# shuoli0708/LRS-PnP-DIP

Measured on AMD Instinct MI355X. Metric: PnP-ISTA+DIP iters/sec on 200×200×198 HSI cube; MPSNR vs reference, higher is better.
Workload: dtype f32 (MFMA products fp32-accurate) + f64 (NLM prox, BN/sigma statistics)

## Files before the change

### include/lrspnp.h

```cpp
#ifndef LRSPNP_H
#define LRSPNP_H

#include <stddef.h>
#include <stdint.h>

#ifdef __cplusplus
extern "C" {
#endif

#define LRS_OK 0
#define LRS_E_INVALID (-1)
#define LRS_E_UNSUPPORTED (-2)
#define LRS_E_WORKSPACE (-3)
#define LRS_E_NODEVICE (-4)

#define LRS_ALPHA_SPEC2 0
#define LRS_ALPHA_FRO4 1
#define LRS_ALPHA_SOFT 2
#define LRS_PROX_NLM 0
#define LRS_PROX_SOFT 1
#define LRS_PROX_NLM_MATLAB 2

const char *lrs_version(void);
int lrs_check_device(void);

int lrs_nlm_col_f32(const float *g, int64_t ldg, float *out, int64_t ldo, int64_t K, int64_t nvec,
                    double h, const double *h_per_vec, int patch_size, int patch_distance,
                    void *stream);

int64_t lrs_block_count(int64_t P, int64_t B, int64_t bb, int64_t sliding);
int lrs_block_grid(int64_t P, int64_t B, int64_t bb, int64_t sliding, int32_t *rows, int32_t *cols,
                   int64_t nb);
int lrs_cover_ranges(int64_t extent, int64_t bb, const int32_t *starts, int64_t nstarts,
                     int32_t *lo, int32_t *hi);

int lrs_im2col_f32(const float *X, const float *L, float mu, int64_t P, int64_t B, int64_t bb,
                   const int32_t *rows, const int32_t *cols, int64_t nb, int64_t n_pad, float *Yb,
                   uint8_t *obs, void *stream);

size_t lrs_ista_alpha_workspace(int64_t n, int64_t K, int64_t npat);
int lrs_ista_alpha_f32(const float *D, int64_t n, int64_t K, const uint8_t *obs_pat, int64_t npat,
                       int64_t n_pad, int alpha_mode, float lambda_ista, float *alpha_pat,
                       double *thr_pat, void *ws, size_t ws_bytes, void *stream);

#define LRS_ISTA_F32 0
#define LRS_ISTA_SPLIT_BF16 1
#define LRS_ISTA_ALGO_AUTO 0
#define LRS_ISTA_ALGO_GENERIC 1
typedef struct {
    int32_t precision;
    int32_t max_workgroups;
    int32_t algorithm;
    int32_t warm_start;
    int32_t reserved[4];
} lrs_ista_opts;
size_t lrs_ista_workspace(int64_t n, int64_t K, int prox, const lrs_ista_opts *opts);
int lrs_ista_f32(const float *Yb, const uint8_t *obs, const float *D, int64_t n, int64_t n_pad,
                 int64_t K, int64_t nb, const float *alpha, const double *thr, int Nit, int prox,
                 float *coefs, float *phi, const lrs_ista_opts *opts, void *ws, size_t ws_bytes,
                 void *stream);
int64_t lrs_ista_pat_plan_len(int64_t nb, int64_t npat);
int64_t lrs_ista_pat_plan(const int32_t *pat, int64_t nb, int64_t npat, int32_t *plan, int64_t cap);
int lrs_ista_pat_preferred(int64_t n, int64_t K, int64_t nb, int64_t npat, int Nit);
size_t lrs_ista_pat_workspace(int64_t n, int64_t K, int64_t npat);
int lrs_ista_pat_prepare(const float *D, int64_t n, int64_t K, const uint8_t *obs_pat, int64_t npat,
                         int64_t n_pad, void *ws, size_t ws_bytes, void *stream);
int lrs_ista_pat_f32(const float *Yb, const uint8_t *obs_pat, int64_t npat, const int32_t *plan,
                     int64_t ntiles, int64_t n, int64_t n_pad, int64_t K, int64_t nb,
                     const float *alpha, const double *thr, int Nit, int prox, float *coefs, float *phi,
                     const lrs_ista_opts *opts, void *ws, size_t ws_bytes, void *stream);
size_t lrs_dict_workspace(int64_t n, int64_t n_pad, int64_t K, int64_t nb);
int lrs_dict_stats_f32(const float *coefs, int64_t nb, int64_t K, float *H, double *c, void *ws,
                       size_t ws_bytes, void *stream);
int lrs_dict_update_f32(const float *Yb, const uint8_t *obs, const float *coefs, float *D, int64_t n,
                        int64_t n_pad, int64_t K, int64_t nb, const double *c, int n_inner, double *obj,
                        void *ws, size_t ws_bytes, void *stream);
int lrs_dict_normalise_f32(float *D, int64_t n, int64_t K, void *stream);
int lrs_nlm_matlab_col_f32(const float *g, int64_t ldg, float *out, int64_t ldo, int64_t K,
                           int64_t nvec, double h, const double *h_per_vec, void *stream);
#define LRS_DIP_F32 0
#define LRS_DIP_SPLIT_BF16 1
typedef struct {
    int32_t precision;
    int32_t upsample_dgrad;
    int32_t reserved[6];
} lrs_dip_opts;

#define LRS_SVT_WARM 1
#define LRS_SVT_JACOBI 2
#define LRS_SVT_MULTI_WG 4
#define LRS_SVT_WIDE_TRI 8
#define LRS_SVT_WIDE_MW 16
int64_t lrs_svt_max_bands(void);
size_t lrs_svt_workspace(int64_t P, int64_t B);
int lrs_svt_f32(const float *X, const float *L2, float c2, int64_t P, int64_t B, double tau,
                float *U, double *s_out, int warm, void *ws, size_t ws_bytes, void *stream);
int lrs_svt_gram_f32(const float *X, const float *L2, float c2, int64_t P, int64_t B, int warm,
                     void *ws, size_t ws_bytes, void *stream);
int lrs_svt_finish_f32(const float *X, const float *L2, float c2, int64_t P, int64_t B, double tau,
                       float *U, double *s_out, int warm, void *ws, size_t ws_bytes, void *stream);
int lrs_svt_gram_offset(int64_t P, int64_t B, int64_t *offset_bytes, int64_t *ld);

int lrs_admm_update_f32(float *X, float *L1, float *L2, const float *Y, const float *M,
                        const float *U, const float *phi, int64_t P, int64_t B, int64_t bb,
                        int64_t n_pad, const int32_t *row_starts, const int32_t *col_starts,
                        int64_t nbr, const int32_t *rlo, const int32_t *rhi, const int32_t *clo,
                        const int32_t *chi, float gamma, float mu1, float mu2, double *norms,
                        float *imout, void *stream);

#define LRS_PAD_ZERO 0
#define LRS_PAD_REFLECT 1
#define LRS_ACT_NONE 0
#define LRS_ACT_LRELU 1
#define LRS_ACT_SIGMOID 2

int lrs_conv2d_out_size(int H, int W, int k, int stride, int pad, int upsample, int *Ho, int *Wo);
int64_t lrs_conv2d_col_size(int Cin, int H, int W, int k, int stride, int pad, int upsample);
size_t lrs_conv2d_workspace(int Cin, int H, int W, int Cout, int k, int stride, int pad, int upsample,
                            const lrs_dip_opts *opts);
int lrs_conv2d_fwd_f32(const float *x, int Cin, int H, int W, const float *w, const float *bias,
                       int Cout, int k, int stride, int pad, int pad_mode, int upsample, float *col,
                       float *y, const lrs_dip_opts *opts, void *ws, size_t ws_bytes, void *stream);
int lrs_conv2d_bwd_f32(const float *gy, const float *col, const float *w, const float *w_div, int Cin,
                       int H, int W, int Cout, int k, int stride, int pad, int pad_mode, int upsample,
                       float *gx, float *gw, const lrs_dip_opts *opts, void *ws, size_t ws_bytes,
                       void *stream);
int lrs_conv2d_bwd_x_f32(const float *gy, const float *x, const float *w, const float *w_div, int Cin,
                         int H, int W, int Cout, int k, int stride, int pad, int pad_mode, int upsample,
                         float *gx, float *gw, const lrs_dip_opts *opts, void *ws, size_t ws_bytes,
                         void *stream);

size_t lrs_bn_act_workspace(int C, int64_t P);
int lrs_bn_act_fwd_f32(const float *z, float *y, const float *gamma, const float *beta, float *mean,
                       float *invstd, float *run_mean, float *run_var, int C, int64_t P, int act,
                       float eps, float momentum, void *ws, size_t ws_bytes, void *stream);
int lrs_bn_act_bwd_f32(const float *gy, const float *y, const float *z, const float *gamma,
                       const float *mean, const float *invstd, float *gz, float *ggamma,
                       float *gbeta, float *gbias, int C, int64_t P, int act, void *ws, size_t ws_bytes,
                       void *stream);
int lrs_conv_bn_small_f32(const float *x, int Cin, int H, int W, const float *w, const float *bias, int Cout,
                          int k, int stride, int pad, int pad_mode, int upsample, const float *gamma,
                          const float *beta, int lip, int act, float *z, float *y, float *mean, float *invstd,
                          float *run_mean, float *run_var, void *stream);

size_t lrs_sigma_max_workspace(int n);
int lrs_sigma_max_f32(const float *const *W, float *const *Wn, const int *rows, const int *cols, int n,
                      float ln_lambda, float *sigma, float *scale, void *ws, size_t ws_bytes,
                      void *stream);

int lrs_adam_f32(float *p, const float *g, float *m, float *v, int64_t n, const int *step, float lr,
                 float beta1, float beta2, float eps, void *stream);
int lrs_masked_mse_f32(const float *out, const float *target, const float *mask, int C, int64_t P,
                       float *gout, double *loss_acc, void *stream);
int lrs_masked_mse_cmask_f32(const float *out, const float *target, const float *mask, int mask_channels,
                             int C, int64_t P, float *gout, double *loss_acc, void *stream);
int lrs_masked_mse_framed_f32(const float *out, const float *target, const float *mask, int mask_channels,
                              int C, int64_t P, int64_t n_mean, float *gout, double *loss_acc, void *stream);

int lrs_unfolded_to_image_f32(const float *X, const float *L, float c, int64_t H, int64_t W, int64_t B,
                              float *img, void *stream);
int lrs_image_to_unfolded_f32(const float *img, int64_t H, int64_t W, int64_t B, float *X, void *stream);
int lrs_unfolded_to_frame_f32(const float *X, const float *L, float c, int64_t H, int64_t W, int64_t B,
                              int64_t top, int64_t left, int64_t Hf, int64_t Wf, float *img, void *stream);
int lrs_frame_to_unfolded_f32(const float *img, int64_t H, int64_t W, int64_t B, int64_t top, int64_t left,
                              int64_t Hf, int64_t Wf, float *X, void *stream);

typedef struct {
    int32_t count, size, patience, wait, stop, stop_epoch, best_epoch, reserved;
// ... 64 lines not shown
```

### lrs-pnp-dip_amd/csrc/dip_launch.h

```cpp
#pragma once
#include <math.h>
#include <string.h>

#include <algorithm>
#include <new>
#include <vector>

#include "dip_kernels.h"
#include "dip_bn.h"
#include "dip_sn.h"
#include "dip_train.h"
#include "dip_gemm.h"
#include "dip_pw.h"
#include "dip_wprep.h"
#include "dip_dgrad.h"
#include "dip_sm.h"
#include "dip_dir.h"
#include "dip_image.h"
#include "ista_paths.h"

using namespace lrs;

namespace {

constexpr int kEw = 256;
constexpr int64_t kForkBigP = 9604;

inline unsigned ew_blocks(int64_t n, int64_t cap = 4096) {
    int64_t b = (n + kEw - 1) / kEw;
    if (b < 1) b = 1;
    if (b > cap) b = cap;
    return (unsigned)b;
}

inline lrs_dip_opts dip_opts(const lrs_dip_opts *o) {
    lrs_dip_opts d{};
    d.precision = LRS_DIP_SPLIT_BF16;
    d.upsample_dgrad = 0;
    return o ? *o : d;
}
inline bool dip_opts_ok(const lrs_dip_opts &o) {
    return (o.precision == LRS_DIP_F32 || o.precision == LRS_DIP_SPLIT_BF16) && (o.upsample_dgrad == 0 || o.upsample_dgrad == 1);
}

int make_geom(int Cin, int H, int W, int k, int stride, int pad, int pad_mode, int up, ConvGeom &g,
              const lrs_dip_opts *opts = nullptr) {
    const lrs_dip_opts o = dip_opts(opts);
    if (!dip_opts_ok(o)) return LRS_E_INVALID;
    if (Cin <= 0 || H <= 0 || W <= 0 || k <= 0 || stride <= 0 || pad < 0) return LRS_E_INVALID;
    if (pad_mode != LRS_PAD_ZERO && pad_mode != LRS_PAD_REFLECT) return LRS_E_INVALID;
    g.Cin = Cin; g.Hs = H; g.Ws = W;
    g.up = up ? 1 : 0; g.Hu = up ? 2 * H : H; g.Wu = up ? 2 * W : W;
    g.pad = pad; g.pad_mode = pad_mode; g.k = k; g.stride = stride;
    if (pad_mode == LRS_PAD_REFLECT && (pad >= g.Hu || pad >= g.Wu)) return LRS_E_INVALID;
    const int hp = g.Hu + 2 * pad, wp = g.Wu + 2 * pad;
    if (hp < k || wp < k) return LRS_E_INVALID;
    g.Ho = (hp - k) / stride + 1;
    g.Wo = (wp - k) / stride + 1;
    g.prec = o.precision;
    g.ke = 0;
    if (o.upsample_dgrad && g.up && g.stride == 1 && g.Hs >= 2 && g.Ws >= 2) {
        if (g.k == 3 && g.pad == 1) g.ke = 4;
        if (g.k == 2 && g.pad == 0) g.ke = 3;
    }
    return LRS_OK;
}

inline bool plain_unit(const ConvGeom &g) { return g.k == 1 && g.stride == 1 && g.pad == 0 && !g.up; }

struct Split { int S, kchunk; bool big; };

constexpr int64_t kSplitMinTiles = 256;
constexpr int kSplitCap = 64;

Split choose_split(int M, int N, int K, int precision = LRS_DIP_SPLIT_BF16, bool force_big = false, int target = 512) {
    const int64_t t128 = (int64_t)((M + kBM - 1) / kBM) * ((N + kBN - 1) / kBN);
    const bool deep = precision == LRS_DIP_SPLIT_BF16 && K >= 65536;
    const bool big = force_big || t128 >= 64 || (precision == LRS_DIP_SPLIT_BF16 && K >= 8192 && t128 >= 4) || deep;
    const int64_t tiles = big ? t128 : (int64_t)((M + kBM64 - 1) / kBM64) * ((N + kBN64 - 1) / kBN64);
    int S = 1;
    if (tiles < kSplitMinTiles) {
        S = (int)((target + tiles - 1) / tiles);
        const int smax = deep ? K / 512 : (K + 127) / 128;
        if (S > smax) S = smax;
        if (S > (deep ? 256 : kSplitCap)) S = deep ? 256 : kSplitCap;
        if (S < 1) S = 1;
    }
    const int bk = (big && precision == LRS_DIP_SPLIT_BF16) ? kBK32 : kBK;
    int kchunk = (int)round_up((K + S - 1) / S, bk);
    if (kchunk < bk) kchunk = bk;
    S = (K + kchunk - 1) / kchunk;
    if (S < 1) S = 1;
    return {S, kchunk, big};
}

int64_t s3_part_floats(int M, int N, int K) {
    const Split s = choose_split(M, N, K, LRS_DIP_SPLIT_BF16, true);
    return s.S > 1 ? (int64_t)s.S * M * N : 0;
}

int64_t gemm_part_floats(int M, int N, int K) {
    const Split a = choose_split(M, N, K, LRS_DIP_F32), b = choose_split(M, N, K, LRS_DIP_SPLIT_BF16);
    const int S = std::max(a.S, b.S);
    return S > 1 ? (int64_t)S * M * N : 0;
}

inline void split_reduce(const Split &s, const float *part, int M, int N, const float *bias, const float *div, int accum,
                         float *C, hipStream_t st) {
    if (s.S > 1)
        hipLaunchKernelGGL(k_gemm_reduce, dim3((unsigned)(((int64_t)M * N + kEw - 1) / kEw)), dim3(kEw), 0, st, part, s.S, M,
                           N, bias, div, accum, C);
}

template <class Launch>
int split_launch(const Split &s, int64_t pcols, float *part, int64_t part_cap, GemmArgs g, dim3 tiles, int zmul,
                 int *nsplit_out, hipStream_t st, Launch launch, bool to_part = false) {
    if (nsplit_out) *nsplit_out = s.S;
    float *C = g.C;
    if (s.S > 1 || to_part) {
        if (!part || part_cap < (int64_t)s.S * g.M * pcols) return LRS_E_WORKSPACE;
        g.C = part;
    }
    launch(g, dim3(tiles.x, tiles.y, (unsigned)(zmul * s.S)));
    if (!nsplit_out && !to_part) split_reduce(s, part, g.M, (int)pcols, g.bias, g.div, g.accum, C, st);
    LRS_CHECK_LAUNCH();
    return LRS_OK;
}

int gemm(int prec, int TA, int TB, const float *A, const float *B, float *C, const float *bias, const float *div, int M,
         int N, int K, float *part, int64_t part_cap, hipStream_t st, int accum = 0, int *nsplit_out = nullptr,
         bool force_big = false, int target = 512) {
    if (M <= 0 || N <= 0) return LRS_OK;
    const Split s = choose_split(M, N, K, prec, force_big, target);
    const int t = (TA ? 2 : 0) + (TB ? 1 : 0);
    static void (*const k128[4])(GemmArgs) = {k_gemm<0, 0>, k_gemm<0, 1>, k_gemm<1, 0>, k_gemm<1, 1>};
    static void (*const k64[4])(GemmArgs) = {k_gemm64<0, 0>, k_gemm64<0, 1>, k_gemm64<1, 0>, k_gemm64<1, 1>};
    const dim3 tiles = s.big ? dim3((N + kBN - 1) / kBN, (M + kBM - 1) / kBM)
                             : dim3((N + kBN64 - 1) / kBN64, (M + kBM64 - 1) / kBM64);
    const auto launch = [&](const GemmArgs &g, dim3 grid) {
        if (s.big && prec == LRS_DIP_SPLIT_BF16) {
            const int lda = TA ? M : K, ldb = TB ? K : N;
#define LRS_S3(RA, RB)                                                                                        \
// ... 148 lines not shown
    const auto launch = [&](const GemmArgs &g, dim3 grid) {
        hipLaunchKernelGGL((k_gemm_s3<LA, LB>), grid, dim3(kGemmThreads), 0, st, g, la, lb);
    };
    return split_launch(s, N, part, part_cap, a, dim3((N + 127) / 128, (M + 127) / 128), 1, nsplit_out, st, launch);
}

int upc_fwd(const ConvGeom &g, const float *x, const __bf16 *wpre, const float *bias, int Cout, float *y, float *part,
            int64_t part_cap, hipStream_t st, int *nsplit_out) {
    const int Cp = r16(g.Cin), Q = g.Hs * g.Ws, K = 4 * Cp;
    const int64_t P = (int64_t)g.Ho * g.Wo;
    const Split s = choose_split(Cout, 4 * Q, K, LRS_DIP_SPLIT_BF16, true, nsplit_out ? kFwdSplitWg : 512);
    const GemmArgs a{nullptr, nullptr, y, bias, nullptr, Cout, Q, K, s.kchunk, 0, 4, g.Ws, g.Wo, P};
    const auto launch = [&](const GemmArgs &ga, dim3 grid) {
        hipLaunchKernelGGL((k_gemm_s3<LdPre, LdUpFwdTM>), grid, dim3(kGemmThreads), 0, st, ga,
                           LdPre{wpre, (int64_t)4 * Cout * K, K, Cout, (int64_t)Cout * K},
                           LdUpFwdTM{x, g.Cin * Q * 4, g, Cp, nullptr});
    };
    return split_launch(s, P, part, part_cap, a, dim3((Q + 127) / 128, (Cout + 127) / 128), 4, nsplit_out, st, launch);
}

int upc_dgrad(const ConvGeom &g, const float *gz, const __bf16 *wd, int Cout, float *gx, float *gxe, float *part,
              int64_t part_cap, hipStream_t st, int accum) {
    const int Cop = r16(Cout), K = 16 * Cop, Qe = (g.Hs + 2) * (g.Ws + 2);
    int nsplit = 1;
    int rc = gemm_s3_conv(LdPre{wd, (int64_t)g.Cin * K, K, g.Cin}, LdUpDgradTM{gz, Cout * g.Ho * g.Wo * 4, g, Cout, Cop, nullptr},
                          gxe, nullptr, nullptr, g.Cin, Qe, K, part, part_cap, st, &nsplit, 0,
                          kDgradSplitWg);
    if (rc) return rc;
    ConvGeom fg = g;
    fg.up = 0;
    fg.Hu = g.Hs;
    fg.Wu = g.Ws;
    fg.pad = 1;
    fg.pad_mode = kPadClamp;
    const dim3 grid((unsigned)((g.Hs * g.Ws + 255) / 256), (unsigned)std::min(g.Cin, 65535));
    hipLaunchKernelGGL(k_fold_pad, grid, dim3(256), 0, st, nsplit > 1 ? part : gxe, nsplit, (int64_t)g.Cin * Qe, fg, gx,
                       accum);
    LRS_CHECK_LAUNCH();
    return LRS_OK;
}

int upc_wgrad(const ConvGeom &g, const float *gz, const float *x, const float *div, int Cout, float *gw, float *part,
              int64_t part_cap, hipStream_t st, int target = 512) {
    const int Q = g.Hs * g.Ws, N = 4 * g.Cin;
    const Split s = choose_split(Cout, 4 * N, Q, LRS_DIP_SPLIT_BF16, true, target);
    const GemmArgs a{nullptr, nullptr, part, nullptr, nullptr, Cout, N, Q, s.kchunk, 0, 4, g.Ws, 0, 0};
    const auto launch = [&](const GemmArgs &ga, dim3 grid) {
        hipLaunchKernelGGL((k_gemm_s3<LdGzCls, LdWgradCls>), grid, dim3(kGemmThreads), 0, st, ga,
                           LdGzCls{gz, g.Hs, g.Ws, g.Wo, Cout, 0}, LdWgradCls{x, g.Cin * Q * 4, g, nullptr, 0, 0});
    };
    const int rc = split_launch(s, 4 * N, part, part_cap, a, dim3((N + 127) / 128, (Cout + 127) / 128), 4, nullptr, st, launch,
                                true);
    if (rc) return rc;
    const int64_t n = (int64_t)Cout * g.Cin * 9;
    hipLaunchKernelGGL(k_upc_wgrad_combine, dim3((unsigned)((n + 255) / 256)), dim3(256), 0, st, part, s.S, Cout, g.Cin,
                       div, gw);
    LRS_CHECK_LAUNCH();
    return LRS_OK;
}

inline bool conv_implicit_ok(const ConvGeom &g, int Cout) {
    return g.k <= 3 && (int64_t)g.Cin * g.Hs * g.Ws * 4 < kOob && (int64_t)Cout * g.Ho * g.Wo * 4 < kOob;
}

constexpr int64_t kImplicitMinP = 1024;

int wprep(const ConvGeom &g, const float *w, int Cout, __bf16 *wf, __bf16 *wd, hipStream_t st) {
    const int kk = g.k * g.k;
    const int64_t elems = wprep_elems(g, Cout, false).total();
    if (elems >= INT32_MAX / 3) return LRS_E_UNSUPPORTED;
    const int64_t n = elems / 3;
    const ConvPrep c{w, nullptr, wf, wd, Cout, g.Cin, kk, r16(g.Cin), r16(Cout), -1, g.k, wd ? g.ke : 0};
    hipLaunchKernelGGL(k_conv_prep1, dim3(ew_blocks(n, 2048)), dim3(256), 0, st, c);
    return LRS_OK;
}

struct PwKernel {
    int mt, nb, wg_per_cu;
    void (*fn)(PwArgs);
};
static const PwKernel kPwKernels[] = {
    {1, 4, 6, k_pw<1, 4>}, {2, 4, 3, k_pw<2, 4>}, {3, 4, 2, k_pw<3, 4>}, {4, 4, 2, k_pw<4, 4>}, {4, 5, 2, k_pw<4, 5>},
};

struct PwHead {
    const float *tgt, *msk;
    int64_t mstride;
    float *gz;
    double *hpart;
    float norm;
    int *nwg_out;
};

int pw_launch(const __bf16 *A, int64_t pstride, int lda, int M, const float *B, int K, int64_t N, float *C,
              const float *bias, int accum, hipStream_t st, int act = 0, const PwHead *head = nullptr) {
    if (M <= 0 || N <= 0) return LRS_OK;
    if (M > 256 || lda < K || lda % 16) return LRS_E_UNSUPPORTED;
    const int Kp32 = (int)round_up(lda, 32), ldsrow = pw_ldsrow(Kp32);
    static std::atomic<uint64_t> attr_set[sizeof(kPwKernels) / sizeof(kPwKernels[0])];
    for (size_t i = 0; i < sizeof(kPwKernels) / sizeof(kPwKernels[0]); ++i)
        if (const int rc = lds_opt_in((const void *)kPwKernels[i].fn, 3 * 80 * pw_ldsrow(256), attr_set[i])) return rc;
    if (Kp32 > 256 || (int64_t)K * N * 4 >= kOob || 3 * pstride * 2 >= kOob) return LRS_E_UNSUPPORTED;
    const PwArgs a{A, pstride, lda, B, K, N, C, bias, M, Kp32, ldsrow, accum, act};
    const int mt = (M + 63) / 64;
    const PwKernel *best = nullptr;
    int64_t best_cost = 0;
    for (const PwKernel &k : kPwKernels) {
        if (k.mt != mt) continue;
        const int lds = 3 * 16 * k.nb * ldsrow;
        const int per_cu = std::min(k.wg_per_cu, (160 * 1024) / lds);
        const int64_t wgs = (N + 16 * k.nb - 1) / (16 * k.nb);
        const int64_t rounds = (wgs + 256 * per_cu - 1) / (256 * per_cu);
        const int64_t cost = rounds * k.nb;
        if (!best || cost < best_cost || (cost == best_cost && k.nb > best->nb)) {
            best = &k;
            best_cost = cost;
        }
    }
    if (!best) return LRS_E_UNSUPPORTED;
    const int npx = 16 * best->nb;
    PwArgs ah = a;
    if (head) {
        ah.tgt = head->tgt;
        ah.msk = head->msk;
        ah.mstride = head->msk ? head->mstride : 0;
        ah.gz = head->gz;
        ah.hpart = head->hpart;
        ah.hnorm = head->norm;
        *head->nwg_out = (int)((N + npx - 1) / npx);
    }
    hipLaunchKernelGGL(best->fn, dim3((unsigned)((N + npx - 1) / npx)), dim3(256), 3 * npx * ldsrow, st, ah);
    LRS_CHECK_LAUNCH();
    return LRS_OK;
}

inline bool pw_ok(const ConvGeom &g, int Cout) { return plain_unit(g) && Cout <= 256 && r16(g.Cin) <= 256 && r16(Cout) <= 256; }

int conv_fwd(const ConvGeom &g, const float *x, const float *w, const float *bias, int Cout, float *col, float *y,
             float *part, int64_t part_cap, hipStream_t st, const __bf16 *wpre = nullptr, int *nsplit_out = nullptr,
             int act_pw = 0, const PwHead *head = nullptr) {
    const int P = g.Ho * g.Wo, Kc = g.Cin * g.k * g.k;
    if (nsplit_out) *nsplit_out = 1;
    const float *B = x;
    if (plain_unit(g) && wpre)
        return pw_launch(wpre, (int64_t)Cout * r16(g.Cin), r16(g.Cin), Cout, x, g.Cin, P, y, bias, 0, st, act_pw, head);
    if (head) return LRS_E_UNSUPPORTED;
    if (!plain_unit(g) && !col) {
        if (!conv_implicit_ok(g, Cout) || !wpre) return LRS_E_UNSUPPORTED;
        const int kk = g.k * g.k, Cp = r16(g.Cin);
        return gemm_s3_conv(LdPre{wpre, (int64_t)Cout * kk * Cp, kk * Cp, Cout},
                            LdFwdTM{x, g.Cin * g.Hs * g.Ws * 4, g, Cp, nullptr}, y, bias, nullptr, Cout, P, kk * Cp,
                            part, part_cap, st, nsplit_out, 0, nsplit_out ? kFwdSplitWg : 512);
    }
    if (!plain_unit(g)) {
        const dim3 grid((unsigned)((P + 255) / 256), (unsigned)std::min(Kc, 65535));
        hipLaunchKernelGGL(k_im2col, grid, dim3(256), 0, st, x, g, col);
        B = col;
    }
    return gemm(g.prec, 0, 0, w, B, y, bias, nullptr, Cout, P, Kc, part, part_cap, st, 0, nsplit_out);
}

int conv_wgrad(const ConvGeom &g, const float *gz, const float *col, const float *div, int Cout, float *gw, float *part,
               int64_t part_cap, hipStream_t st, bool implicit, int *wsplit_out = nullptr, int wtarget = 512) {
    const int P = g.Ho * g.Wo, Kc = g.Cin * g.k * g.k;
    if (implicit && !plain_unit(g)) {
        if (!conv_implicit_ok(g, Cout)) return LRS_E_UNSUPPORTED;
        return gemm_s3_conv(LdDense<true>{gz, P, Cout}, LdWgradTM{col, g.Cin * g.Hs * g.Ws * 4, g, nullptr, 0}, gw,
                            nullptr, div, Cout, Kc, P, part, part_cap, st, wsplit_out, 0, wtarget);
    }
    return gemm(g.prec, 0, 1, gz, col, gw, nullptr, div, Cout, Kc, P, part, part_cap, st, 0, wsplit_out, plain_unit(g),
                wtarget);
}


int dgrad_pointwise(const ConvGeom &g, const float *gz, const float *w, const __bf16 *wpre, int Cout, float *gx,
                    float *part, int64_t part_cap, hipStream_t st, int accum) {
    const int P = g.Ho * g.Wo;
    if (wpre)
        return pw_launch(wpre + wprep_elems(g, Cout, false).fwd, (int64_t)g.Cin * r16(Cout), r16(Cout), g.Cin, gz, Cout, P,
                         gx, nullptr, accum, st);
    return gemm(g.prec, 1, 0, w, gz, gx, nullptr, nullptr, g.Cin, P, Cout, part, part_cap, st, accum);
}

int dgrad_effective(const ConvGeom &g, const float *gz, const float *w, const __bf16 *we, int Cout, float *gx,
                    float *border, float *part, int64_t part_cap, hipStream_t st) {
    const int P = g.Ho * g.Wo, ke = g.ke, Cop = r16(Cout), ke2 = ke * ke;
    ConvGeom ge{};
    ge.Cin = Cout; ge.Hs = g.Ho; ge.Ws = g.Wo; ge.up = 0; ge.Hu = g.Ho; ge.Wu = g.Wo;
    ge.pad = 1; ge.pad_mode = LRS_PAD_ZERO; ge.k = ke; ge.stride = 2; ge.Ho = g.Hs; ge.Wo = g.Ws;
    if ((g.Ho + 2 - ke) / 2 + 1 != g.Hs || (g.Wo + 2 - ke) / 2 + 1 != g.Ws) return LRS_E_INVALID;
    const int rc = gemm_s3_conv(LdPre{we, (int64_t)g.Cin * ke2 * Cop, ke2 * Cop, g.Cin},
                                LdFwdTM{gz, Cout * P * 4, ge, Cop, nullptr}, gx, nullptr, nullptr, g.Cin, g.Hs * g.Ws,
                                ke2 * Cop, part, part_cap, st);
    if (rc) return rc;
    if (g.pad_mode == LRS_PAD_REFLECT && g.k == 3) {
        const int Lmax = std::max(g.Ws, g.Hs);
        float *S = border, *corr = border + (int64_t)4 * 3 * Cout * Lmax;
        hipLaunchKernelGGL(k_up_border_s, dim3((unsigned)((12 * Lmax + 255) / 256), (unsigned)Cout), dim3(256), 0, st,
                           gz, Cout, g.Hs, g.Ws, Lmax, S);
        hipLaunchKernelGGL(k_up_border_mm, dim3(4, (unsigned)((g.Cin + kUbC - 1) / kUbC), (unsigned)((Lmax + 127) / 128)),
                           dim3(256), 0, st, S, w, g.Cin, Cout, g.Hs, g.Ws, Lmax, corr);
        const int nper = 2 * g.Ws + 2 * (g.Hs - 2);
        hipLaunchKernelGGL(k_up_border_add, dim3((unsigned)((nper + 255) / 256), (unsigned)g.Cin), dim3(256), 0, st,
                           corr, g.Cin, g.Hs, g.Ws, Lmax, gx);
    }
    LRS_CHECK_LAUNCH();
    return LRS_OK;
}

int dgrad_padded(const ConvGeom &g, const float *gz, const __bf16 *wd, int Cout, float *gx, float *dcol, float *part,
                 int64_t part_cap, hipStream_t st, int accum) {
    const int P = g.Ho * g.Wo, kk = g.k * g.k, Cop = r16(Cout), Qp = (g.Hu + 2 * g.pad) * (g.Wu + 2 * g.pad);
    int nsplit = 1;
    const int rc = gemm_s3_conv(LdPre{wd, (int64_t)g.Cin * kk * Cop, kk * Cop, g.Cin},
                                LdDgradTM{gz, Cout * P * 4, g, Cout, Cop, nullptr}, dcol, nullptr, nullptr, g.Cin, Qp,
                                kk * Cop, part, part_cap, st, &nsplit, 0, kDgradSplitWg);
    if (rc) return rc;
    if (nsplit == 1 && !g.up && g.Ws % 4 == 0 && g.Cin <= 65535 && ((uintptr_t)gx & 15) == 0) {
        const int q = g.Hs * (g.Ws / 4);
        hipLaunchKernelGGL(k_fold_pad1q, dim3((unsigned)((q + 255) / 256), (unsigned)g.Cin), dim3(256), 0, st, dcol,
                           g, gx, accum);
    } else {
        const dim3 grid((unsigned)((g.Hs * g.Ws + 255) / 256), (unsigned)std::min(g.Cin, 65535));
        hipLaunchKernelGGL(k_fold_pad, grid, dim3(256), 0, st, nsplit > 1 ? part : dcol, nsplit, (int64_t)g.Cin * Qp,
                           g, gx, accum);
    }
    LRS_CHECK_LAUNCH();
    return LRS_OK;
}

int dgrad_col2im(const ConvGeom &g, const float *gz, const float *w, int Cout, float *gx, float *dcol, float *part,
                 int64_t part_cap, hipStream_t st, int accum) {
    const int P = g.Ho * g.Wo, Kc = g.Cin * g.k * g.k;
    const int rc = gemm(g.prec, 1, 0, w, gz, dcol, nullptr, nullptr, Kc, P, Cout, part, part_cap, st);
    if (rc) return rc;
    const dim3 grid((unsigned)((g.Hs * g.Ws + 255) / 256), (unsigned)std::min(g.Cin, 65535));
    if (g.stride == 1) hipLaunchKernelGGL(k_col2im<1>, grid, dim3(256), 0, st, dcol, g, gx, accum);
    else if (g.stride == 2) hipLaunchKernelGGL(k_col2im<2>, grid, dim3(256), 0, st, dcol, g, gx, accum);
    else hipLaunchKernelGGL(k_col2im<0>, grid, dim3(256), 0, st, dcol, g, gx, accum);
    LRS_CHECK_LAUNCH();
    return LRS_OK;
}

int conv_dgrad(const ConvGeom &g, const float *gz, const float *w, int Cout, float *gx, float *dcol, float *part,
               int64_t part_cap, hipStream_t st, int accum, bool implicit, const __bf16 *wpre) {
    if (plain_unit(g)) return dgrad_pointwise(g, gz, w, wpre, Cout, gx, part, part_cap, st, accum);
    const __bf16 *wd = (implicit && wpre) ? wpre + wprep_elems(g, Cout, false).fwd : nullptr;
    const int P = g.Ho * g.Wo, Kc = g.Cin * g.k * g.k;
    const bool refl_border = g.pad_mode == LRS_PAD_REFLECT && g.k == 3;
    const bool border_fits = dcol && (int64_t)4 * (3 * Cout + g.Cin) * std::max(g.Ws, g.Hs) <= (int64_t)Kc * P;
    if (wd && g.ke && !accum && (!refl_border || border_fits))
        return dgrad_effective(g, gz, w, wd, Cout, gx, dcol, part, part_cap, st);
    if (!dcol) return LRS_E_WORKSPACE;
    const int Qp = (g.Hu + 2 * g.pad) * (g.Wu + 2 * g.pad);
    if (wd && g.stride == 1 && (int64_t)g.Cin * Qp <= (int64_t)Kc * P)
        return dgrad_padded(g, gz, wd, Cout, gx, dcol, part, part_cap, st, accum);
    return dgrad_col2im(g, gz, w, Cout, gx, dcol, part, part_cap, st, accum);
}

inline bool al16(const void *p) { return ((uintptr_t)p & 15) == 0; }

int bn_fwd(const float *z, float *y, const float *gamma, const float *beta, float *mean, float *invstd, float *rm,
           float *rv, int C, int64_t P, int act, float eps, float mom, double *part, hipStream_t st, int lip = 1) {
    const int S = bn_split(P);
    const int vec = (P % 4 == 0 && al16(z) && al16(y)) ? 1 : 0;
    int chunk = (int)((P + S - 1) / S);
    if (vec) chunk = (chunk + 3) & ~3;
    BnArgs a{z, y, gamma, beta, mean, invstd, rm, rv, part, C, (int)P, S, chunk, gamma ? 1 : 0, act, eps, mom, lip,
             vec};
    if (const int nq = gamma ? bn_reg_q(P, vec) : 0) {
        launch_bn_fwd_r(nq, nullptr, 0, nullptr, a, nullptr, st);
    } else if (gamma && bn_one_wg(P)) {
        hipLaunchKernelGGL(k_bn_fwd1, dim3(1, C), dim3(bn1_threads(P)), 0, st, a);
    } else {
        if (gamma) hipLaunchKernelGGL(k_bn_stats, dim3(S, C), dim3(kBnThreads), 0, st, a);
        hipLaunchKernelGGL(k_bn_apply, dim3(S, C), dim3(kBnThreads), 0, st, a);
    }
    LRS_CHECK_LAUNCH();
    return LRS_OK;
}

int bn_bwd(const float *gy, const float *y, const float *z, const float *gamma, const float *mean,
           const float *invstd, float *gz, float *ggamma, float *gbeta, float *gbias, int C, int64_t P, int act,
           double *part, hipStream_t st, int lip = 1, int accum = 0, const float *beta = nullptr) {
    const int S = bn_split(P);
    const int vec = (P % 4 == 0 && al16(gy) && al16(y) && al16(z) && al16(gz)) ? 1 : 0;
    int chunk = (int)((P + S - 1) / S);
    if (vec) chunk = (chunk + 3) & ~3;
    BnBwdArgs a{gy, y, z, gamma, mean, invstd, gz, ggamma, gbeta, gbias, part, C, (int)P, S, chunk,
                gamma ? 1 : 0, act, lip, accum, vec, gamma ? beta : nullptr};
    if (const int nq = gamma ? bn_reg_q(P, vec) : 0) {
        launch_bn_bwd_r(nq, a, st);
    } else if ((gamma || gbias) && bn_one_wg(P)) {
        hipLaunchKernelGGL(k_bn_bwd1, dim3(1, C), dim3(bn1_threads(P)), 0, st, a);
    } else {
        if (gamma || gbias) hipLaunchKernelGGL(k_bn_bwd_stats, dim3(S, C), dim3(kBnThreads), 0, st, a);
        hipLaunchKernelGGL(k_bn_bwd_apply, dim3(S, C), dim3(kBnThreads), 0, st, a);
    }
    LRS_CHECK_LAUNCH();
    return LRS_OK;
}

void dir_launch(const ConvGeom &g, const DirGeom &dg, const float *x, const float *w, const float *bias, const BnArgs &a,
                hipStream_t st) {
    const dim3 grid(1, a.C);
#define LRS_DIR(KS, S)                                                                                         \
    do {                                                                                                        \
        if (dg.vec4) hipLaunchKernelGGL((k_conv_bn_dir<KS, S, true>), grid, dim3(kDirTh), 0, st, x, w, bias, g, dg, a); \
        else hipLaunchKernelGGL((k_conv_bn_dir<KS, S, false>), grid, dim3(kDirTh), 0, st, x, w, bias, g, dg, a);     \
    } while (0)
    if (g.k == 3 && g.stride == 1) LRS_DIR(3, 1);
    else if (g.k == 3) LRS_DIR(3, 2);
    else if (g.stride == 1) LRS_DIR(1, 1);
    else LRS_DIR(1, 2);
#undef LRS_DIR
}

int sn_launch(const SnConv *table_dev, int n, int64_t max_elems, double *gram, float *sigma, float *scale,
              float ln_lambda, bool apply, hipStream_t st, long long *prof = nullptr) {
    hipLaunchKernelGGL(k_sn_gram, dim3(kSnSplit, n), dim3(256), 0, st, table_dev, gram);
    hipLaunchKernelGGL(k_sn_gram_reduce, dim3(kSnPairs, n), dim3(256), 0, st, table_dev, gram);
    hipLaunchKernelGGL(k_sn_sigma, dim3(n), dim3(256), 0, st, table_dev, gram, sigma, scale, ln_lambda, prof);
    if (apply) hipLaunchKernelGGL(k_sn_apply, dim3(ew_blocks(max_elems, 256), n), dim3(kEw), 0, st, table_dev, scale);
    LRS_CHECK_LAUNCH();
    return LRS_OK;
}

int es_update(const float *out, int64_t N, float *ring, lrs_es_state *es, hipStream_t st, const EsCrop *cr = nullptr) {
    const unsigned nblk = ew_blocks(N, kEsMaxBlocks);
    if (cr) {
        if (N > INT32_MAX) return LRS_E_UNSUPPORTED;
        hipLaunchKernelGGL(k_es_step_crop, dim3(nblk), dim3(kEw), 0, st, out, N, ring, es, *cr);
    } else {
        hipLaunchKernelGGL(k_es_step, dim3(nblk), dim3(kEw), 0, st, out, N, ring, es);
    }
    hipLaunchKernelGGL(k_es_decide, dim3(1), dim3(64), 0, st, (const float *)ring, N, (int)nblk, es);
    LRS_CHECK_LAUNCH();
    return LRS_OK;
}

}
```

### lrs-pnp-dip_amd/csrc/dip_pw.h

```cpp
#pragma once

#include "dip_kernels.h"
#include "dip_gemm.h"

namespace lrs {

struct PwArgs {
    const __bf16 *A;
    int64_t pstride;
    int lda;
    const float *B;
    int K;
    int64_t N;
    float *C;
    const float *bias;
    int M, Kp32, ldsrow, accum;
    int act;
    const float *tgt = nullptr, *msk = nullptr;
    int64_t mstride = 0;
    float *gz = nullptr;
    double *hpart = nullptr;
    float hnorm = 0.0f;
};

// ... 120 lines not shown
#pragma unroll
            for (int r = 0; r < 4; ++r) E[(4 * gk + r) * ES + 16 * b + jl] = acc[j][b][r];
        __builtin_amdgcn_s_waitcnt(0xc07f);
        __builtin_amdgcn_wave_barrier();
        double hs[NB], hb[NB];
#pragma unroll
        for (int i = 0; i < NB; ++i) {
            hs[i] = 0.0;
            hb[i] = 0.0;
            const int idx = lane + 64 * i, rr = idx / (4 * NB), q = 4 * (idx % (4 * NB));
            const int m = 16 * wv + 64 * j + rr;
            const int64_t n = n0 + q;
            if (m >= a.M) continue;
            float4 v = *reinterpret_cast<const float4 *>(E + rr * ES + q);
            const float bs = a.bias ? a.bias[m] : 0.0f;
            float *c = a.C + (int64_t)m * a.N + n;
            if (vec && n + 3 < a.N) {
                if (a.bias) { v.x = v.x + bs; v.y = v.y + bs; v.z = v.z + bs; v.w = v.w + bs; }
                if (a.accum) {
                    const float4 o = *reinterpret_cast<const float4 *>(c);
                    v.x = o.x + v.x; v.y = o.y + v.y; v.z = o.z + v.z; v.w = o.w + v.w;
                }
                if (a.act) { v.x = act_fwd(v.x, a.act); v.y = act_fwd(v.y, a.act); v.z = act_fwd(v.z, a.act); v.w = act_fwd(v.w, a.act); }
                *reinterpret_cast<float4 *>(c) = v;
                if (head) {
                    const float4 tv = *reinterpret_cast<const float4 *>(a.tgt + (int64_t)m * a.N + n);
                    const float4 mv = a.msk ? *reinterpret_cast<const float4 *>(a.msk + (int64_t)m * a.mstride + n)
                                            : make_float4(1.0f, 1.0f, 1.0f, 1.0f);
                    const float oe[4] = {v.x, v.y, v.z, v.w}, te[4] = {tv.x, tv.y, tv.z, tv.w}, me[4] = {mv.x, mv.y, mv.z, mv.w};
                    float ge[4];
#pragma unroll
                    for (int e = 0; e < 4; ++e) {
                        const float d = te[e] * me[e] - oe[e] * me[e];
                        hs[i] += (double)d * (double)d;
                        ge[e] = act_bwd((-(a.hnorm * d)) * me[e], oe[e], a.act);
                        hb[i] += (double)ge[e];
                    }
                    *reinterpret_cast<float4 *>(a.gz + (int64_t)m * a.N + n) = make_float4(ge[0], ge[1], ge[2], ge[3]);
                }
            } else {
                const float vv[4] = {v.x, v.y, v.z, v.w};
                for (int u = 0; u < 4; ++u) {
                    if (n + u >= a.N) break;
                    float x = vv[u];
                    if (a.bias) x = x + bs;
                    if (a.accum) x = c[u] + x;
                    if (a.act) x = act_fwd(x, a.act);
                    c[u] = x;
                    if (head) {
                        const float mk = a.msk ? a.msk[(int64_t)m * a.mstride + n + u] : 1.0f;
                        const float d = a.tgt[(int64_t)m * a.N + n + u] * mk - x * mk;
                        hs[i] += (double)d * (double)d;
                        const float g = act_bwd((-(a.hnorm * d)) * mk, x, a.act);
                        a.gz[(int64_t)m * a.N + n + u] = g;
                        hb[i] += (double)g;
                    }
                }
            }
        }
        __builtin_amdgcn_wave_barrier();
        if (head) {
            double2 *R = reinterpret_cast<double2 *>(E);
            static_assert(16 * 4 * NB * sizeof(double2) <= 16 * ES * sizeof(float), "head sums fit the staging");
#pragma unroll
            for (int i = 0; i < NB; ++i) R[lane + 64 * i] = make_double2(hs[i], hb[i]);
            __builtin_amdgcn_s_waitcnt(0xc07f);
            __builtin_amdgcn_wave_barrier();
            const int m = 16 * wv + 64 * j + lane;
            if (lane < 16 && m < a.M) {
                double sl = 0.0, sg = 0.0;
                for (int k = 0; k < 4 * NB; ++k) {
                    const double2 p = R[lane * 4 * NB + k];
                    sl += p.x;
                    sg += p.y;
                }
                a.hpart[(int64_t)m * gridDim.x + blockIdx.x] = sg;
                a.hpart[((int64_t)a.M + m) * gridDim.x + blockIdx.x] = sl;
            }
            __builtin_amdgcn_wave_barrier();
        }
    }
}

__global__ __launch_bounds__(256) void k_head_reduce(const double *__restrict__ hpart, int C, int nwg, float *gbias,
                                                     double *closs) {
    __shared__ double red[12];
    const int c = blockIdx.x;
    double sg = 0.0, sl = 0.0;
    for (int w = threadIdx.x; w < nwg; w += blockDim.x) {
        sg += hpart[(int64_t)c * nwg + w];
        sl += hpart[((int64_t)C + c) * nwg + w];
    }
    block_sum2_d(sg, sl, red);
    if (threadIdx.x == 0) {
        gbias[c] = (float)sg;
        closs[c] = sl;
    }
}

__global__ void k_head_loss(const double *__restrict__ closs, int C, double *loss_acc) {
    if (threadIdx.x != 0 || blockIdx.x != 0) return;
    double s = 0.0;
    for (int c = 0; c < C; ++c) s += closs[c];
    *loss_acc += s;
}

}
```

### lrs-pnp-dip_amd/csrc/lrs_dip.h

```cpp
#pragma once
#include "lrs_common.h"

namespace lrs {

struct ConvGeom {
    int Cin, Hs, Ws, up, Hu, Wu, pad, pad_mode, k, stride, Ho, Wo;
    int prec, ke;
};

struct SnConv {
    const float *W;
    float *Wn;
    int rows, cols;
};

}
```

### lrs-pnp-dip_amd/lrspnp/_lib.py

```python
from __future__ import annotations

import ctypes
import os

_HERE = os.path.dirname(os.path.abspath(__file__))
LIB_PATH = os.environ.get("LRSPNP_LIB") or os.path.join(_HERE, "liblrspnp_hip.so")
CSRC = os.path.join(os.path.dirname(_HERE), "csrc")

LRS_OK = 0
LRS_E = {-1: "LRS_E_INVALID", -2: "LRS_E_UNSUPPORTED", -3: "LRS_E_WORKSPACE", -4: "LRS_E_NODEVICE"}

ALPHA_SPEC2, ALPHA_FRO4, ALPHA_SOFT = 0, 1, 2
PROX_NLM, PROX_SOFT, PROX_NLM_MATLAB = 0, 1, 2


class LrsError(RuntimeError):
    pass


ISTA_F32, ISTA_SPLIT_BF16 = 0, 1
DIP_F32, DIP_SPLIT_BF16 = 0, 1


ISTA_ALGO_AUTO, ISTA_ALGO_GENERIC = 0, 1

SVT_WARM, SVT_JACOBI, SVT_MULTI_WG, SVT_WIDE_TRI, SVT_WIDE_MW = 1, 2, 4, 8, 16


class IstaOpts(ctypes.Structure):
    _fields_ = [("precision", ctypes.c_int32), ("max_workgroups", ctypes.c_int32), ("algorithm", ctypes.c_int32),
                ("warm_start", ctypes.c_int32), ("reserved", ctypes.c_int32 * 4)]


class DipOpts(ctypes.Structure):
    _fields_ = [("precision", ctypes.c_int32), ("upsample_dgrad", ctypes.c_int32), ("reserved", ctypes.c_int32 * 6)]


def ista_opts(precision: int = ISTA_SPLIT_BF16, max_workgroups: int = 0, algorithm: int = ISTA_ALGO_AUTO,
              warm_start: int = 0) -> IstaOpts:
    return IstaOpts(precision=precision, max_workgroups=max_workgroups, algorithm=algorithm, warm_start=warm_start)


def dip_opts(precision: int = DIP_SPLIT_BF16, upsample_dgrad: int = 0) -> DipOpts:
    return DipOpts(precision=precision, upsample_dgrad=upsample_dgrad)


_lib = None
_device_checked = False
_PER_BAND_MASK = ("lrs_masked_mse_cmask_f32", "lrs_dipnet_train_steps_cmask")
_FRAME = ("lrs_masked_mse_framed_f32", "lrs_unfolded_to_frame_f32", "lrs_frame_to_unfolded_f32",
          "lrs_dipnet_set_frame", "lrs_dipnet_get_frame")


def build(force: bool = False) -> str:
    import subprocess

    if force:
        subprocess.check_call(["make", "-s", "-C", CSRC, "clean"])
    subprocess.check_call(["make", "-s", "-j8", "-C", CSRC])
    return LIB_PATH


def _declare(L):
    c = ctypes
    vp, i64, i32, f32, f64, sz = c.c_void_p, c.c_int64, c.c_int, c.c_float, c.c_double, c.c_size_t
    i32p = c.POINTER(c.c_int32)
    dop = c.POINTER(DipOpts)
    sig = {
        "lrs_version": (c.c_char_p, []),
        "lrs_check_device": (i32, []),
        "lrs_nlm_col_f32": (i32, [vp, i64, vp, i64, i64, i64, f64, vp, i32, i32, vp]),
        "lrs_block_count": (i64, [i64, i64, i64, i64]),
        "lrs_block_grid": (i32, [i64, i64, i64, i64, i32p, i32p, i64]),
        "lrs_cover_ranges": (i32, [i64, i64, i32p, i64, i32p, i32p]),
        "lrs_im2col_f32": (i32, [vp, vp, f32, i64, i64, i64, vp, vp, i64, i64, vp, vp, vp]),
        "lrs_ista_alpha_workspace": (sz, [i64, i64, i64]),
        "lrs_ista_alpha_f32": (i32, [vp, i64, i64, vp, i64, i64, i32, f32, vp, vp, vp, sz, vp]),
        "lrs_ista_workspace": (sz, [i64, i64, i32, c.POINTER(IstaOpts)]),
        "lrs_ista_f32": (i32, [vp, vp, vp, i64, i64, i64, i64, vp, vp, i32, i32, vp, vp, c.POINTER(IstaOpts), vp,
                               sz, vp]),
        "lrs_nlm_matlab_col_f32": (i32, [vp, i64, vp, i64, i64, i64, f64, vp, vp]),
        "lrs_ista_pat_plan_len": (i64, [i64, i64]),
        "lrs_ista_pat_plan": (i64, [i32p, i64, i64, i32p, i64]),
        "lrs_ista_pat_preferred": (i32, [i64, i64, i64, i64, i32]),
        "lrs_ista_pat_workspace": (sz, [i64, i64, i64]),
        "lrs_ista_pat_prepare": (i32, [vp, i64, i64, vp, i64, i64, vp, sz, vp]),
        "lrs_ista_pat_f32": (i32, [vp, vp, i64, vp, i64, i64, i64, i64, i64, vp, vp, i32, i32, vp, vp,
                                   c.POINTER(IstaOpts), vp, sz, vp]),
        "lrs_dict_workspace": (sz, [i64, i64, i64, i64]),
        "lrs_dict_stats_f32": (i32, [vp, i64, i64, vp, vp, vp, sz, vp]),
        "lrs_dict_update_f32": (i32, [vp, vp, vp, vp, i64, i64, i64, i64, vp, i32, vp, vp, sz, vp]),
        "lrs_dict_normalise_f32": (i32, [vp, i64, i64, vp]),
        "lrs_ssim_f32":(i32, [vp, vp, i32, i32, i32, vp, vp]),
        "lrs_psnr_workspace": (sz, [i64, i64]),
        "lrs_psnr_bands_f32": (i32, [vp, vp, i64, i64, vp, vp, sz, vp]),
        "lrs_svt_max_bands": (i64, []),
        "lrs_svt_workspace": (sz, [i64, i64]),
        "lrs_svt_f32": (i32, [vp, vp, f32, i64, i64, f64, vp, vp, i32, vp, sz, vp]),
        "lrs_svt_gram_f32": (i32, [vp, vp, f32, i64, i64, i32, vp, sz, vp]),
        "lrs_svt_finish_f32": (i32, [vp, vp, f32, i64, i64, f64, vp, vp, i32, vp, sz, vp]),
        "lrs_svt_gram_offset": (i32, [i64, i64, vp, vp]),
        "lrs_diag_svt_state": (i32, [vp, i64, i64, vp]),
        "lrs_diag_svt_apply": (i32, [vp, vp, f32, i64, i64, vp, vp, vp]),
        "lrs_admm_update_f32": (i32, [vp, vp, vp, vp, vp, vp, vp, i64, i64, i64, i64, vp, vp, i64, vp, vp,
                                      vp, vp, f32, f32, f32, vp, vp, vp]),
        "lrs_conv2d_out_size": (i32, [i32, i32, i32, i32, i32, i32, c.POINTER(c.c_int), c.POINTER(c.c_int)]),
        "lrs_conv2d_col_size": (i64, [i32, i32, i32, i32, i32, i32, i32]),
        "lrs_conv2d_workspace": (sz, [i32, i32, i32, i32, i32, i32, i32, i32, dop]),
        "lrs_conv2d_fwd_f32": (i32, [vp, i32, i32, i32, vp, vp, i32, i32, i32, i32, i32, i32, vp, vp, dop, vp, sz,
                                     vp]),
        "lrs_conv2d_bwd_f32": (i32, [vp, vp, vp, vp, i32, i32, i32, i32, i32, i32, i32, i32, i32, vp, vp, dop, vp,
                                     sz, vp]),
        "lrs_conv2d_bwd_x_f32": (i32, [vp, vp, vp, vp, i32, i32, i32, i32, i32, i32, i32, i32, i32, vp, vp, dop, vp,
                                       sz, vp]),
        "lrs_bn_act_workspace": (sz, [i32, i64]),
        "lrs_bn_act_fwd_f32": (i32, [vp, vp, vp, vp, vp, vp, vp, vp, i32, i64, i32, f32, f32, vp, sz, vp]),
        "lrs_bn_act_bwd_f32": (i32, [vp, vp, vp, vp, vp, vp, vp, vp, vp, vp, i32, i64, i32, vp, sz, vp]),
        "lrs_conv_bn_small_f32": (i32, [vp, i32, i32, i32, vp, vp, i32, i32, i32, i32, i32, i32, vp, vp, i32, i32,
                                        vp, vp, vp, vp, vp, vp, vp]),
        "lrs_sigma_max_workspace": (sz, [i32]),
        "lrs_sigma_max_f32": (i32, [c.POINTER(vp), c.POINTER(vp), c.POINTER(c.c_int), c.POINTER(c.c_int), i32,
                                    f32, vp, vp, vp, sz, vp]),
        "lrs_diag_sigma_phases": (i32, [c.POINTER(vp), c.POINTER(c.c_int), c.POINTER(c.c_int), i32, vp, sz, vp, vp]),
        "lrs_adam_f32": (i32, [vp, vp, vp, vp, i64, vp, f32, f32, f32, f32, vp]),
        "lrs_masked_mse_f32": (i32, [vp, vp, vp, i32, i64, vp, vp, vp]),
        "lrs_masked_mse_cmask_f32": (i32, [vp, vp, vp, i32, i32, i64, vp, vp, vp]),
        "lrs_unfolded_to_image_f32": (i32, [vp, vp, f32, i64, i64, i64, vp, vp]),
# ... 73 lines not shown
```

Measured before the change: 8.425.

## Add streaming pointwise-conv kernel for small-M large-P 1x1 convolutions

Adds a new k_pws kernel for 1x1 convolution GEMMs with M<=128. Each workgroup handles a 64-column strip of the activation matrix and splits it into bf16x3 parts in double-buffered LDS, runs split MFMA, and writes fp32 output through an LDS staging buffer. It is picked automatically when P exceeds 4096 and alignment holds, or forced through a new pw_stream option, in place of the existing tiled pw kernels. It adds a new kernel variant and more LDS use per workgroup, which could lower occupancy.

After: 8.418, median of 3. About the same (-0.1%).

```diff
diff --git a/include/lrspnp.h b/include/lrspnp.h
--- a/include/lrspnp.h
+++ b/include/lrspnp.h
@@ -83,7 +83,8 @@
 typedef struct {
     int32_t precision;
     int32_t upsample_dgrad;
-    int32_t reserved[6];
+    int32_t pw_stream;
+    int32_t reserved[5];
 } lrs_dip_opts;
 
 #define LRS_SVT_WARM 1
diff --git a/lrs-pnp-dip_amd/csrc/dip_launch.h b/lrs-pnp-dip_amd/csrc/dip_launch.h
--- a/lrs-pnp-dip_amd/csrc/dip_launch.h
+++ b/lrs-pnp-dip_amd/csrc/dip_launch.h
@@ -40,7 +40,8 @@
     return o ? *o : d;
 }
 inline bool dip_opts_ok(const lrs_dip_opts &o) {
-    return (o.precision == LRS_DIP_F32 || o.precision == LRS_DIP_SPLIT_BF16) && (o.upsample_dgrad == 0 || o.upsample_dgrad == 1);
+    return (o.precision == LRS_DIP_F32 || o.precision == LRS_DIP_SPLIT_BF16) && (o.upsample_dgrad == 0 || o.upsample_dgrad == 1) &&
+           (o.pw_stream == 0 || o.pw_stream == 1);
 }
 
 int make_geom(int Cin, int H, int W, int k, int stride, int pad, int pad_mode, int up, ConvGeom &g,
@@ -58,6 +59,7 @@
     g.Ho = (hp - k) / stride + 1;
     g.Wo = (wp - k) / stride + 1;
     g.prec = o.precision;
+    g.pws = o.pw_stream;
     g.ke = 0;
     if (o.upsample_dgrad && g.up && g.stride == 1 && g.Hs >= 2 && g.Ws >= 2) {
         if (g.k == 3 && g.pad == 1) g.ke = 4;
@@ -372,6 +374,17 @@
 static const PwKernel kPwKernels[] = {
     {1, 4, 6, k_pw<1, 4>}, {2, 4, 3, k_pw<2, 4>}, {3, 4, 2, k_pw<3, 4>}, {4, 4, 2, k_pw<4, 4>}, {4, 5, 2, k_pw<4, 5>},
 };
+typedef void (*PwFn)(PwArgs);
+#define LRS_PWS_ROW(MT) {k_pws<MT, 1>, k_pws<MT, 2>, k_pws<MT, 3>, k_pws<MT, 4>, k_pws<MT, 5>, k_pws<MT, 6>, k_pws<MT, 7>, k_pws<MT, 8>}
+static const PwFn kPwsKernels[2][8] = {LRS_PWS_ROW(1), LRS_PWS_ROW(2)};
+#undef LRS_PWS_ROW
+
+inline bool al16(const void *p) { return ((uintptr_t)p & 15) == 0; }
+
+constexpr int64_t kPwStreamMinP = 4096;
+inline bool pw_stream_ok(int M, int64_t N, const float *C, bool head, bool force) {
+    return M <= 128 && N % 4 == 0 && al16(C) && !head && (force || N > kPwStreamMinP);
+}
 
 struct PwHead {
     const float *tgt, *msk;
@@ -383,7 +396,8 @@
 };
 
 int pw_launch(const __bf16 *A, int64_t pstride, int lda, int M, const float *B, int K, int64_t N, float *C,
-              const float *bias, int accum, hipStream_t st, int act = 0, const PwHead *head = nullptr) {
+              const float *bias, int accum, hipStream_t st, int act = 0, const PwHead *head = nullptr,
+              bool force_stream = false) {
     if (M <= 0 || N <= 0) return LRS_OK;
     if (M > 256 || lda < K || lda % 16) return LRS_E_UNSUPPORTED;
     const int Kp32 = (int)round_up(lda, 32), ldsrow = pw_ldsrow(Kp32);
@@ -393,6 +407,14 @@
     if (Kp32 > 256 || (int64_t)K * N * 4 >= kOob || 3 * pstride * 2 >= kOob) return LRS_E_UNSUPPORTED;
     const PwArgs a{A, pstride, lda, B, K, N, C, bias, M, Kp32, ldsrow, accum, act};
     const int mt = (M + 63) / 64;
+    if (pw_stream_ok(M, N, C, head != nullptr, force_stream)) {
+        const PwFn fn = kPwsKernels[mt - 1][Kp32 / 32 - 1];
+        static std::atomic<uint64_t> sattr_set[2][8];
+        if (const int rc = lds_opt_in((const void *)fn, kPwsLds, sattr_set[mt - 1][Kp32 / 32 - 1])) return rc;
+        hipLaunchKernelGGL(fn, dim3((unsigned)((N + 63) / 64)), dim3(256), kPwsLds, st, a);
+        LRS_CHECK_LAUNCH();
+        return LRS_OK;
+    }
     const PwKernel *best = nullptr;
     int64_t best_cost = 0;
     for (const PwKernel &k : kPwKernels) {
@@ -433,7 +455,8 @@
     if (nsplit_out) *nsplit_out = 1;
     const float *B = x;
     if (plain_unit(g) && wpre)
-        return pw_launch(wpre, (int64_t)Cout * r16(g.Cin), r16(g.Cin), Cout, x, g.Cin, P, y, bias, 0, st, act_pw, head);
+        return pw_launch(wpre, (int64_t)Cout * r16(g.Cin), r16(g.Cin), Cout, x, g.Cin, P, y, bias, 0, st, act_pw, head,
+                         g.pws != 0);
     if (head) return LRS_E_UNSUPPORTED;
     if (!plain_unit(g) && !col) {
         if (!conv_implicit_ok(g, Cout) || !wpre) return LRS_E_UNSUPPORTED;
@@ -468,7 +491,7 @@
     const int P = g.Ho * g.Wo;
     if (wpre)
         return pw_launch(wpre + wprep_elems(g, Cout, false).fwd, (int64_t)g.Cin * r16(Cout), r16(Cout), g.Cin, gz, Cout, P,
-                         gx, nullptr, accum, st);
+                         gx, nullptr, accum, st, 0, nullptr, g.pws != 0);
     return gemm(g.prec, 1, 0, w, gz, gx, nullptr, nullptr, g.Cin, P, Cout, part, part_cap, st, accum);
 }
 
@@ -548,8 +571,6 @@
     return dgrad_col2im(g, gz, w, Cout, gx, dcol, part, part_cap, st, accum);
 }
 
-inline bool al16(const void *p) { return ((uintptr_t)p & 15) == 0; }
-
 int bn_fwd(const float *z, float *y, const float *gamma, const float *beta, float *mean, float *invstd, float *rm,
            float *rv, int C, int64_t P, int act, float eps, float mom, double *part, hipStream_t st, int lip = 1) {
     const int S = bn_split(P);
diff --git a/lrs-pnp-dip_amd/csrc/dip_pw.h b/lrs-pnp-dip_amd/csrc/dip_pw.h
--- a/lrs-pnp-dip_amd/csrc/dip_pw.h
+++ b/lrs-pnp-dip_amd/csrc/dip_pw.h
@@ -226,6 +226,106 @@
     }
 }
 
+constexpr int kPwsRow = 80;
+constexpr int kPwsSlot = 3 * 64 * kPwsRow;
+constexpr int kPwsES = 64 + 4;
+constexpr int kPwsLds = 2 * kPwsSlot + 4 * 16 * kPwsES * 4;
+
+template <int MT, int KS>
+__global__ __launch_bounds__(256, KS <= 4 ? 3 : 2) void k_pws(PwArgs a) {
+    extern __shared__ __attribute__((aligned(16))) char pws_smem[];
+    const int t = threadIdx.x, lane = t & 63, wv = __builtin_amdgcn_readfirstlane(t >> 6), jl = lane & 15, gk = lane >> 4;
+    constexpr int NB = 4;
+    const int64_t n0 = (int64_t)blockIdx.x * 64;
+    const __amdgpu_buffer_rsrc_t rs = s3_rsrc(a.B, (int)(a.K * a.N * 4));
+    const __amdgpu_buffer_rsrc_t ra = s3_rsrc(a.A, (int)(3 * a.pstride * 2));
+    bf16x8 fa[MT][3];
+    auto loadA = [&](int ks) {
+        const int k = ks * 32 + 8 * gk;
+#pragma unroll
+        for (int j = 0; j < MT; ++j) {
+            const int row = 16 * wv + 64 * j + jl;
+            const int vo = (row < a.M && k < a.lda) ? 2 * (row * a.lda + k) : kOob;
+#pragma unroll
+            for (int p = 0; p < 3; ++p)
+                fa[j][p] = __builtin_bit_cast(bf16x8, __builtin_amdgcn_raw_buffer_load_b128(ra, vo, (int)(2 * p * a.pstride), 0));
+        }
+    };
+    loadA(0);
+    float v[KS][8];
+    const int voff = n0 + lane < a.N ? (int)((n0 + lane) * 4) : kOob;
+#pragma unroll
+    for (int ks = 0; ks < KS; ++ks)
+#pragma unroll
+        for (int u = 0; u < 8; ++u) {
+            const int64_t so = (int64_t)(8 * (wv + 4 * ks) + u) * a.N * 4;
+            v[ks][u] = s3_bload(rs, voff, so < kOob ? (int)so : kOob);
+        }
+    float *E = reinterpret_cast<float *>(pws_smem + 2 * kPwsSlot) + wv * 16 * kPwsES;
+    {
+        floatx4 acc[MT][NB];
+#pragma unroll
+        for (int j = 0; j < MT; ++j)
+#pragma unroll
+            for (int b = 0; b < NB; ++b) acc[j][b] = floatx4{0.f, 0.f, 0.f, 0.f};
+#pragma unroll
+        for (int ks = 0; ks < KS; ++ks) {
+            char *ring = pws_smem + (ks & 1) * kPwsSlot;
+            {
+                bf16x8 p0, p1, p2;
+                split_bf16x8(v[ks], p0, p1, p2);
+                char *dst = ring + lane * kPwsRow + 16 * wv;
+                *reinterpret_cast<bf16x8 *>(dst) = p0;
+                *reinterpret_cast<bf16x8 *>(dst + 64 * kPwsRow) = p1;
+                *reinterpret_cast<bf16x8 *>(dst + 2 * 64 * kPwsRow) = p2;
+            }
+            if (ks > 0) loadA(ks);
+            __builtin_amdgcn_s_waitcnt(0xc07f);
+            __builtin_amdgcn_s_barrier();
+            bf16x8 fb[NB][3];
+#pragma unroll
+            for (int b = 0; b < NB; ++b) {
+                const char *s0 = ring + (16 * b + jl) * kPwsRow + 16 * gk;
+#pragma unroll
+                for (int p = 0; p < 3; ++p) fb[b][p] = *reinterpret_cast<const bf16x8 *>(s0 + p * 64 * kPwsRow);
+            }
+#pragma unroll
+            for (int j = 0; j < MT; ++j)
+#pragma unroll
+                for (int b = 0; b < NB; ++b) acc[j][b] = split_mfma6(fa[j], fb[b], acc[j][b]);
+        }
+#pragma unroll
+        for (int j = 0; j < MT; ++j) {
+#pragma unroll
+            for (int b = 0; b < NB; ++b)
+#pragma unroll
+                for (int r = 0; r < 4; ++r) E[(4 * gk + r) * kPwsES + 16 * b + jl] = acc[j][b][r];
+            __builtin_amdgcn_s_waitcnt(0xc07f);
+            __builtin_amdgcn_wave_barrier();
+#pragma unroll
+            for (int i = 0; i < NB; ++i) {
+                const int idx = lane + 64 * i, rr = idx / 16, q = 4 * (idx % 16);
+                const int m = 16 * wv + 64 * j + rr;
+                const int64_t n = n0 + q;
+                if (m >= a.M || n >= a.N) continue;
+                float4 x = *reinterpret_cast<const float4 *>(E + rr * kPwsES + q);
+                float *c = a.C + (int64_t)m * a.N + n;
+                if (a.bias) {
+                    const float bs = a.bias[m];
+                    x.x = x.x + bs; x.y = x.y + bs; x.z = x.z + bs; x.w = x.w + bs;
+                }
+                if (a.accum) {
+                    const float4 o = *reinterpret_cast<const float4 *>(c);
+                    x.x = o.x + x.x; x.y = o.y + x.y; x.z = o.z + x.z; x.w = o.w + x.w;
+                }
+                if (a.act) { x.x = act_fwd(x.x, a.act); x.y = act_fwd(x.y, a.act); x.z = act_fwd(x.z, a.act); x.w = act_fwd(x.w, a.act); }
+                *reinterpret_cast<float4 *>(c) = x;
+            }
+            __builtin_amdgcn_wave_barrier();
+        }
+    }
+}
+
 __global__ __launch_bounds__(256) void k_head_reduce(const double *__restrict__ hpart, int C, int nwg, float *gbias,
                                                      double *closs) {
     __shared__ double red[12];
diff --git a/lrs-pnp-dip_amd/csrc/lrs_dip.h b/lrs-pnp-dip_amd/csrc/lrs_dip.h
--- a/lrs-pnp-dip_amd/csrc/lrs_dip.h
+++ b/lrs-pnp-dip_amd/csrc/lrs_dip.h
@@ -5,7 +5,7 @@
 
 struct ConvGeom {
     int Cin, Hs, Ws, up, Hu, Wu, pad, pad_mode, k, stride, Ho, Wo;
-    int prec, ke;
+    int prec, ke, pws;
 };
 
 struct SnConv {
diff --git a/lrs-pnp-dip_amd/lrspnp/_lib.py b/lrs-pnp-dip_amd/lrspnp/_lib.py
--- a/lrs-pnp-dip_amd/lrspnp/_lib.py
+++ b/lrs-pnp-dip_amd/lrspnp/_lib.py
@@ -33,7 +33,8 @@
 
 
 class DipOpts(ctypes.Structure):
-    _fields_ = [("precision", ctypes.c_int32), ("upsample_dgrad", ctypes.c_int32), ("reserved", ctypes.c_int32 * 6)]
+    _fields_ = [("precision", ctypes.c_int32), ("upsample_dgrad", ctypes.c_int32), ("pw_stream", ctypes.c_int32),
+                ("reserved", ctypes.c_int32 * 5)]
 
 
 def ista_opts(precision: int = ISTA_SPLIT_BF16, max_workgroups: int = 0, algorithm: int = ISTA_ALGO_AUTO,
@@ -41,8 +42,8 @@
     return IstaOpts(precision=precision, max_workgroups=max_workgroups, algorithm=algorithm, warm_start=warm_start)
 
 
-def dip_opts(precision: int = DIP_SPLIT_BF16, upsample_dgrad: int = 0) -> DipOpts:
-    return DipOpts(precision=precision, upsample_dgrad=upsample_dgrad)
+def dip_opts(precision: int = DIP_SPLIT_BF16, upsample_dgrad: int = 0, pw_stream: int = 0) -> DipOpts:
+    return DipOpts(precision=precision, upsample_dgrad=upsample_dgrad, pw_stream=pw_stream)
 
 
 _lib = None
```
